# wq2012/SpectralCluster

Hardware: AMD Instinct MI355X
Metric: predict() calls/sec, n=8192 d=256 ICASSP2018 (GraphCut, eigengap k in [2,20], cosine k-means) (higher is better)
Workload: dtype f64; 1 GPU; icassp2018_graphcut_n8192_d256_k8_max20; n_samples=8192, n_features=256, parallelism=replicas x1, collectives=none

## Files before the change

spectralcluster_amd/csrc/eig.hip:

```cpp
#include <algorithm>
#include <cstring>
#include <mutex>

#include "sc_internal.h"

namespace sc {

typedef double v4f64 __attribute__((ext_vector_type(4)));
constexpr int B = kEigBlock;
constexpr int RB = 256 / B;
static_assert(B == 8 || B == 16, "block width must divide the 16-wide MFMA tile");

__device__ __forceinline__ uint64_t splitmix64(uint64_t x) {
  x += 0x9E3779B97F4A7C15ull;
  x = (x ^ (x >> 30)) * 0xBF58476D1CE4E5B9ull;
  x = (x ^ (x >> 27)) * 0x94D049BB133111EBull;
  return x ^ (x >> 31);
}
__device__ __forceinline__ double hash_uniform(uint64_t seed, uint64_t idx) {
  const uint64_t h = splitmix64(seed ^ splitmix64(idx));
  return (double)(h >> 11) * (2.0 / 9007199254740992.0) - 1.0;
}

__global__ void k_random_block(double* W, int n, uint64_t seed) {
  const int e = blockIdx.x * blockDim.x + threadIdx.x;
  if (e < n * B) W[e] = hash_uniform(seed, (uint64_t)e);
}

__global__ void k_refill_deficient(double* W, int n, const int* flags,
                                   uint64_t seed) {
  const int e = blockIdx.x * blockDim.x + threadIdx.x;
  if (e >= n * B) return;
  if ((flags[0] >> (e & (B - 1))) & 1) W[e] = hash_uniform(seed, (uint64_t)e);
}

constexpr int kMvWaves = 8;
__device__ __forceinline__ void block_matvec_body(
    const double* __restrict__ S, int ld, int n, const double* __restrict__ cvec,
    const double* __restrict__ pvec, const double* __restrict__ V, int ldv,
    const double* __restrict__ Vs, double* __restrict__ W) {
  __shared__ double red[kMvWaves][64][4];
  const int lane = threadIdx.x & 63;
  const int wave = threadIdx.x >> 6;
  const int li = lane & 15, lg = lane >> 4;
  const int r0 = blockIdx.x * 16;
  int ri = r0 + li;
  ri = ri < n ? ri : n - 1;
  const double* srow = S + (size_t)ri * ld + 2 * lg;
  v4f64 acc0 = {0.0, 0.0, 0.0, 0.0}, acc1 = {0.0, 0.0, 0.0, 0.0};
  const int nchunks = (n + 31) / 32;
  double2 cur[4], nxt[4];
  auto load = [&](double2* dst, int ch) {
    const int kb = ch * 32 + 2 * lg;
#pragma unroll
    for (int q = 0; q < 4; ++q) {
      if (kb + 8 * q + 1 < ld)
        dst[q] = *reinterpret_cast<const double2*>(srow + ch * 32 + 8 * q);
      else
        dst[q] = make_double2(0.0, 0.0);
    }
  };
  int ch = wave;
  if (ch < nchunks) load(cur, ch);
  for (; ch < nchunks; ch += kMvWaves) {
    if (ch + kMvWaves < nchunks) load(nxt, ch + kMvWaves);
    const int kb = ch * 32 + 2 * lg;
    double b[8];
#pragma unroll
    for (int t = 0; t < 8; ++t) {
      const int k = kb + 8 * (t >> 1) + (t & 1);
      b[t] = (k < n && li < B) ? Vs[(size_t)k * B + li] : 0.0;
    }
#pragma unroll
    for (int q = 0; q < 4; ++q) {
      const double a0 = (kb + 8 * q < n) ? cur[q].x : 0.0;
      const double a1 = (kb + 8 * q + 1 < n) ? cur[q].y : 0.0;
      acc0 = __builtin_amdgcn_mfma_f64_16x16x4f64(a0, b[2 * q], acc0, 0, 0, 0);
      acc1 = __builtin_amdgcn_mfma_f64_16x16x4f64(a1, b[2 * q + 1], acc1, 0, 0, 0);
    }
#pragma unroll
    for (int q = 0; q < 4; ++q) cur[q] = nxt[q];
  }
#pragma unroll
  for (int r = 0; r < 4; ++r) red[wave][lane][r] = acc0[r] + acc1[r];
  __syncthreads();
  if (wave == 0) {
#pragma unroll
    for (int r = 0; r < 4; ++r) {
      double sum = 0.0;
#pragma unroll
      for (int w = 0; w < kMvWaves; ++w) sum += red[w][lane][r];
      const int row = r0 + lg + 4 * r;
      if (row < n && li < B)
        W[(size_t)row * B + li] =
            __builtin_fma(cvec ? cvec[row] : 1.0, sum,
                          pvec ? pvec[row] * V[(size_t)row * ldv + li] : 0.0);
    }
  }
}
__global__ __launch_bounds__(64 * kMvWaves) void k_block_matvec(
    const double* __restrict__ S, int ld, int n, const double* __restrict__ cvec,
    const double* __restrict__ pvec, const double* __restrict__ V, int ldv,
    const double* __restrict__ Vs, double* __restrict__ W) {
  block_matvec_body(S, ld, n, cvec, pvec, V, ldv, Vs, W);
}
__global__ __launch_bounds__(64 * kMvWaves) void k_block_matvec_g(const GroupOf<MatvecItem> g) {
  const MatvecItem& a = g.s[blockIdx.y];
  if ((int)blockIdx.x * 16 >= a.n) return;
  block_matvec_body(a.S, a.ld, a.n, a.cvec, a.pvec, a.V, a.ldv, a.Vs, a.W);
}

constexpr int kSymTile = 128;
constexpr int kSymPitch = 34;
__device__ __forceinline__ int sym_item_id(int I, int J, int nt) {
  return I * nt - I * (I - 1) / 2 + (J - I);
}
__device__ __forceinline__ void block_matvec_sym_body(
    const double* __restrict__ S, int ld, int n, const double* __restrict__ Vs,
    double* __restrict__ pdirect, double* __restrict__ pmirror, int nt) {
  __shared__ __attribute__((aligned(16))) double smem[4 * 32 * kSymPitch];
  int I = 0, rem = blockIdx.x, rowlen = nt;
  while (rem >= rowlen) {
    rem -= rowlen;
    --rowlen;
    ++I;
  }
  const int J = I + rem;
  const bool diag = I == J;
  const int lane = threadIdx.x & 63, wave = threadIdx.x >> 6;
  const int li = lane & 15, lg = lane >> 4;
  const int r0 = I * kSymTile + 32 * wave;
  const int c0 = J * kSymTile;
  double* patch = smem + wave * (32 * kSymPitch);
  double bm[8];
#pragma unroll
  for (int t = 0; t < 8; ++t) {
    const int row = r0 + 4 * t + lg;
    bm[t] = (row < n && li < B) ? Vs[(size_t)row * B + li] : 0.0;
  }
  v4f64 accd[2] = {{0.0, 0.0, 0.0, 0.0}, {0.0, 0.0, 0.0, 0.0}};
  v4f64 accm[4][2];
#pragma unroll
  for (int cs = 0; cs < 4; ++cs)
#pragma unroll
    for (int ct = 0; ct < 2; ++ct) accm[cs][ct] = (v4f64){0.0, 0.0, 0.0, 0.0};
  double2 a[1][2][4];
  auto load = [&](int buf, int cs) {
#pragma unroll
    for (int rt = 0; rt < 2; ++rt) {
      int row = r0 + 16 * rt + li;
      row = row < n ? row : n - 1;
      const double* src = S + (size_t)row * ld + c0 + 32 * cs + 2 * lg;
#pragma unroll
      for (int q = 0; q < 4; ++q) {
        if (c0 + 32 * cs + 8 * q + 2 * lg + 1 < ld)
          a[buf][rt][q] = *reinterpret_cast<const double2*>(src + 8 * q);
        else
          a[buf][rt][q] = make_double2(0.0, 0.0);
      }
    }
  };
#pragma unroll
  for (int cs = 0; cs < 4; ++cs) {
    constexpr int cur = 0;
    load(cur, cs);
    const int kb = c0 + 32 * cs + 2 * lg;
#pragma unroll
    for (int rt = 0; rt < 2; ++rt) {
      const bool rok = r0 + 16 * rt + li < n;
#pragma unroll
      for (int q = 0; q < 4; ++q) {
        if (!rok || kb + 8 * q >= n) a[cur][rt][q].x = 0.0;
        if (!rok || kb + 8 * q + 1 >= n) a[cur][rt][q].y = 0.0;
      }
    }
    double b[8];
#pragma unroll
    for (int t = 0; t < 8; ++t) {
      const int k = kb + 8 * (t >> 1) + (t & 1);
      b[t] = (k < n && li < B) ? Vs[(size_t)k * B + li] : 0.0;
    }
#pragma unroll
    for (int rt = 0; rt < 2; ++rt)
#pragma unroll
      for (int q = 0; q < 4; ++q) {
        accd[rt] = __builtin_amdgcn_mfma_f64_16x16x4f64(a[cur][rt][q].x, b[2 * q], accd[rt], 0, 0, 0);
        accd[rt] = __builtin_amdgcn_mfma_f64_16x16x4f64(a[cur][rt][q].y, b[2 * q + 1], accd[rt], 0, 0, 0);
      }
    if (!diag) {
#pragma unroll
      for (int rt = 0; rt < 2; ++rt)
#pragma unroll
        for (int q = 0; q < 4; ++q)
          *reinterpret_cast<double2*>(patch + (16 * rt + li) * kSymPitch + 8 * q + 2 * lg) =
              a[cur][rt][q];
      __builtin_amdgcn_fence(__ATOMIC_RELEASE, "wavefront");
      __builtin_amdgcn_wave_barrier();
#pragma unroll
      for (int ct = 0; ct < 2; ++ct)
#pragma unroll
        for (int t = 0; t < 8; ++t) {
          const double at = patch[(4 * t + lg) * kSymPitch + 16 * ct + li];
          accm[cs][ct] = __builtin_amdgcn_mfma_f64_16x16x4f64(at, bm[t], accm[cs][ct], 0, 0, 0);
        }
      __builtin_amdgcn_fence(__ATOMIC_ACQUIRE, "wavefront");
      __builtin_amdgcn_wave_barrier();
    }
  }
  const size_t item = blockIdx.x;
  if (li < B) {
#pragma unroll
    for (int rt = 0; rt < 2; ++rt)
#pragma unroll
      for (int r = 0; r < 4; ++r)
        pdirect[(item * kSymTile + 32 * wave + 16 * rt + lg + 4 * r) * B + li] = accd[rt][r];
  }
  if (diag) return;
  __syncthreads();
  double* red = smem;
  if (li < B) {
#pragma unroll
    for (int cs = 0; cs < 4; ++cs)
#pragma unroll
      for (int ct = 0; ct < 2; ++ct)
#pragma unroll
        for (int r = 0; r < 4; ++r)
          red[(wave * kSymTile + 32 * cs + 16 * ct + lg + 4 * r) * B + li] = accm[cs][ct][r];
  }
  __syncthreads();
  for (int e = threadIdx.x; e < kSymTile * B; e += 256)
    pmirror[item * (kSymTile * B) + e] =
        ((red[e] + red[kSymTile * B + e]) + red[2 * kSymTile * B + e]) + red[3 * kSymTile * B + e];
}
__global__ __launch_bounds__(256) void k_block_matvec_sym(
    const double* __restrict__ S, int ld, int n, const double* __restrict__ Vs,
    double* __restrict__ pdirect, double* __restrict__ pmirror, int nt) {
  block_matvec_sym_body(S, ld, n, Vs, pdirect, pmirror, nt);
}
__global__ __launch_bounds__(256) void k_block_matvec_sym_g(const GroupOf<MatvecItem> g) {
  const MatvecItem& a = g.s[blockIdx.y];
  const int nt = (a.n + kSymTile - 1) / kSymTile;
  if ((int)blockIdx.x >= nt * (nt + 1) / 2) return;
  block_matvec_sym_body(a.S, a.ld, a.n, a.Vs, a.slabs, a.slabs + (size_t)(nt * (nt + 1) / 2) * kSymTile * B, nt);
}

__device__ __forceinline__ void matvec_sym_reduce_body(
    const double* __restrict__ pdirect, const double* __restrict__ pmirror, int nt, int n,
    const double* __restrict__ cvec, const double* __restrict__ pvec,
    const double* __restrict__ V, int ldv, double* __restrict__ W) {
  const int R = blockIdx.x / 4;
  const int e = (blockIdx.x & 3) * 256 + threadIdx.x;
  const int rl = e / B, v = e % B;
  const int row = R * kSymTile + rl;
  double acc = 0.0;
  const int total = nt;
  for (int s0 = 0; s0 < total; s0 += 8) {
    double x[8];
#pragma unroll
    for (int u = 0; u < 8; ++u) {
      const int sidx = s0 + u;
      x[u] = 0.0;
      if (sidx < nt - R) {
        x[u] = pdirect[(size_t)sym_item_id(R, R + sidx, nt) * (kSymTile * B) + e];
      } else if (sidx < total) {
        x[u] = pmirror[(size_t)sym_item_id(sidx - (nt - R), R, nt) * (kSymTile * B) + e];
      }
    }
#pragma unroll
    for (int u = 0; u < 8; ++u) acc += x[u];
  }
  if (row < n) W[(size_t)row * B + v] =
      __builtin_fma(cvec ? cvec[row] : 1.0, acc, pvec ? pvec[row] * V[(size_t)row * ldv + v] : 0.0);
}
__global__ __launch_bounds__(256) void k_matvec_sym_reduce(
    const double* __restrict__ pdirect, const double* __restrict__ pmirror, int nt, int n,
    const double* __restrict__ cvec, const double* __restrict__ pvec,
    const double* __restrict__ V, int ldv, double* __restrict__ W) {
  matvec_sym_reduce_body(pdirect, pmirror, nt, n, cvec, pvec, V, ldv, W);
}
__global__ __launch_bounds__(256) void k_matvec_sym_reduce_g(const GroupOf<MatvecItem> g) {
  const MatvecItem& a = g.s[blockIdx.y];
  const int nt = (a.n + kSymTile - 1) / kSymTile;
  if ((int)blockIdx.x >= nt * 4) return;
  matvec_sym_reduce_body(a.slabs, a.slabs + (size_t)(nt * (nt + 1) / 2) * kSymTile * B, nt, a.n,
                         a.cvec, a.pvec, a.V, a.ldv, a.W);
}

constexpr int kProjGroups = 256 / B;
constexpr int kProjAcc = (kLdq + kProjGroups - 1) / kProjGroups;
__global__ __launch_bounds__(256) void k_proj_partial(
    const double* __restrict__ Q, int ldq, int m, const double* __restrict__ W,
    int n, double* __restrict__ partial) {
  __shared__ double Ql[8][kLdq];
  __shared__ double Wl[8][B];
  const int tid = threadIdx.x;
  const int jj = tid % B, ig = tid / B;
  const int rows_per = (n + gridDim.x - 1) / gridDim.x;
  const int rbeg = blockIdx.x * rows_per;
  const int rend = min(n, rbeg + rows_per);
  double acc[kProjAcc];
#pragma unroll
  for (int q = 0; q < kProjAcc; ++q) acc[q] = 0.0;
  for (int r = rbeg; r < rend; r += 8) {
    __syncthreads();
    for (int e = tid; e < 8 * m; e += 256) {
      const int rr = e / m, i = e - rr * m;
      Ql[rr][i] = (r + rr < rend) ? Q[(size_t)(r + rr) * ldq + i] : 0.0;
    }
    if (tid < 8 * B) {
      const int rr = tid / B;
      Wl[rr][jj] = (r + rr < rend) ? W[(size_t)(r + rr) * B + jj] : 0.0;
    }
    __syncthreads();
#pragma unroll
    for (int rr = 0; rr < 8; ++rr) {
      const double w = Wl[rr][jj];
#pragma unroll
      for (int q = 0; q < kProjAcc; ++q)
        if (ig + kProjGroups * q < m)
          acc[q] = __builtin_fma(Ql[rr][ig + kProjGroups * q], w, acc[q]);
    }
  }
  double* out = partial + (size_t)blockIdx.x * (kLdq * B);
#pragma unroll
  for (int q = 0; q < kProjAcc; ++q)
    if (ig + kProjGroups * q < m) out[(ig + kProjGroups * q) * B + jj] = acc[q];
}

__global__ __launch_bounds__(256) void k_reduce_H(
    const double* __restrict__ partial, int nparts, int m, double* __restrict__ Hbuf,
    double* __restrict__ T, int ldt, int col0, int accumulate,
    double* __restrict__ hsq) {
  __shared__ double sq[32];
  const int tid = threadIdx.x;
  const int sub = tid & 7;
  const int e = blockIdx.x * 32 + (tid >> 3);
  double h = 0.0;
  if (e < m * B)
    for (int g = sub; g < nparts; g += 8) h += partial[(size_t)g * (kLdq * B) + e];
  h += __shfl_xor(h, 1);
  h += __shfl_xor(h, 2);
  h += __shfl_xor(h, 4);
  if (sub == 0) {
    if (e < m * B) {
      Hbuf[e] = h;
      if (T != nullptr) {
        const int i = e / B, j = col0 + (e % B);
        if (i <= j) {
          const double v = accumulate ? T[(size_t)i * ldt + j] + h : h;
          T[(size_t)i * ldt + j] = v;
          T[(size_t)j * ldt + i] = v;
        }
      }
    } else {
      h = 0.0;
    }
    sq[tid >> 3] = h * h;
  }
  __syncthreads();
  if (tid < B) {
    double s = 0.0;
    for (int q = tid; q < 32; q += B) s += sq[q];
    atomicAdd(&hsq[tid], s);
  }
}

__global__ __launch_bounds__(256) void k_update_block(
    const double* __restrict__ Q, int ldq, int m, const double* __restrict__ Hbuf,
    double* __restrict__ W, int n) {
  __shared__ double Hl[kLdq * B];
  __shared__ double Ql[RB][kLdq + 1];
  const int tid = threadIdx.x;
  const int jj = tid % B, rr = tid / B;
  const int r0 = blockIdx.x * RB;
  for (int e = tid; e < m * B; e += 256) Hl[e] = Hbuf[e];
  for (int e = tid; e < RB * m; e += 256) {
    const int a = e / m, i = e - a * m;
    Ql[a][i] = (r0 + a < n) ? Q[(size_t)(r0 + a) * ldq + i] : 0.0;
  }
  __syncthreads();
  const int r = r0 + rr;
  if (r < n) {
    double acc = W[(size_t)r * B + jj];
    for (int i = 0; i < m; ++i) acc = __builtin_fma(-Ql[rr][i], Hl[i * B + jj], acc);
    W[(size_t)r * B + jj] = acc;
  }
}

__device__ __forceinline__ void chol8_wave(const double* G, double* __restrict__ Rinv,
                                           const double* __restrict__ hsq,
                                           int* __restrict__ flags,
                                           int* __restrict__ defect_flag, int flag_mode,
                                           int* __restrict__ sticky_flag = nullptr,
                                           int sticky_m = 0, bool sticky_on_defect = true);

__global__ __launch_bounds__(256) void k_reduce_chol(
    const double* __restrict__ partial, int nparts, double* __restrict__ Rinv,
    double* __restrict__ Gsave, const double* __restrict__ hsq,
    int* __restrict__ flags, int* __restrict__ defect_flag, int flag_mode) {
  static_assert(B == 8, "the factorisation below maps the 8 x 8 matrix onto one wavefront");
  __shared__ double G[B * B];
  const int tid = threadIdx.x;
  {
    constexpr int kLanes = 256 / (B * B);
    const int e = tid / kLanes, sub = tid % kLanes;
    double g = 0.0;
    for (int q = sub; q < nparts; q += kLanes) g += partial[(size_t)q * (kLdq * B) + e];
#pragma unroll
    for (int o = 1; o < kLanes; o <<= 1) g += __shfl_xor(g, o);
    if (sub == 0) {
      G[e] = g;
      if (Gsave) Gsave[e] = g;
    }
  }
  __syncthreads();
  if (tid >= 64) return;
  chol8_wave(G, Rinv, hsq, flags, defect_flag, flag_mode);
}

__device__ __forceinline__ void chol8_wave(const double* G, double* __restrict__ Rinv,
                                           const double* __restrict__ hsq,
                                           int* __restrict__ flags,
                                           int* __restrict__ defect_flag, int flag_mode,
                                           int* __restrict__ sticky_flag, int sticky_m,
                                           bool sticky_on_defect) {
  const int tid = threadIdx.x;
  const int i = tid >> 3, j = tid & 7;
  double g = G[tid];
  const double gii = __shfl(g, i * 9), gjj = __shfl(g, j * 9);
  double defect = 0.0;
  if (flag_mode == 2 && gii != 0.0 && gjj != 0.0) defect = fabs(g - (i == j ? 1.0 : 0.0));
#pragma unroll
  for (int o = 1; o < 64; o <<= 1) defect = fmax(defect, __shfl_xor(defect, o));
  double r = 0.0;
  int mask = 0;
  double pmax = 0.0, pmin = __builtin_huge_val();
#pragma unroll
  for (int k = 0; k < B; ++k) {
    const double d = __shfl(g, k * 9);
    const double total = __shfl(gii, k * 8) + (hsq ? hsq[k] : 0.0);
    const bool drop = !(d > 1e-22 * total) || !(d > 0.0);
    const double rk = drop ? 0.0 : sqrt(d);
    if (drop) {
      mask |= 1 << k;
    } else {
      pmax = fmax(pmax, rk);
      pmin = fmin(pmin, rk);
    }
    double row = 0.0;
    if (i == k && !drop) row = j == k ? rk : (j > k ? g / rk : 0.0);
    if (i == k) r = row;
    const double rki = __shfl(row, k * 8 + i), rkj = __shfl(row, k * 8 + j);
    if (i > k && j > k) g -= rki * rkj;
  }
  const double rii = __shfl(r, i * 9), rjj = __shfl(r, j * 9);
  double ri = 0.0;
#pragma unroll
  for (int srow = B - 1; srow >= 0; --srow) {
    double v = 0.0;
#pragma unroll
    for (int k = srow + 1; k < B; ++k) {
      const double rsk = __shfl(r, srow * 8 + k), rkj = __shfl(ri, k * 8 + j);
      if (k <= j) v -= rsk * rkj;
    }
    if (i == srow && j >= i && rii != 0.0 && rjj != 0.0)
      ri = i == j ? 1.0 / rii : v / rii;
  }
  Rinv[tid] = ri;
  if (tid == 0 && flags != nullptr) {
    flags[0] = mask;
    if (defect_flag != nullptr) *defect_flag = (defect > 0.1 || pmax > 1e3 * pmin) ? 1 : 0;
    if (sticky_flag != nullptr && (mask != 0 || (sticky_on_defect && defect > 0.1))) {
      if (*sticky_flag == 0) {
        sticky_flag[1] = sticky_m;
        sticky_flag[2] = flag_mode * 1000 + mask;
      }
      *sticky_flag = 1;
    }
  }
}

__global__ __launch_bounds__(256) void k_apply_rinv(
    double* __restrict__ W, int n, const double* __restrict__ Rinv,
    double* __restrict__ Qdst, int ldq, int col0, const double* __restrict__ cvec,
    double* __restrict__ Vs) {
  __shared__ double Rl[B * B];
  const int tid = threadIdx.x;
  if (tid < B * B) Rl[tid] = Rinv[tid];
  __syncthreads();
  const int jj = tid % B;
  const int r = blockIdx.x * RB + tid / B;
  const double w = r < n ? W[(size_t)r * B + jj] : 0.0;
  double v = 0.0;
#pragma unroll
  for (int k = 0; k < B; ++k) {
    const double wk = __shfl(w, k, B);
    v = __builtin_fma(wk, Rl[k * B + jj], v);
  }
  if (r < n) {
    W[(size_t)r * B + jj] = v;
    if (Qdst) Qdst[(size_t)r * ldq + col0 + jj] = v;
    if (Vs) Vs[(size_t)r * B + jj] = cvec[r] * v;
  }
}

constexpr int kLzThreads = 512;
constexpr int kLzPartStride = (kLdq + B) * B;
struct LzStep {
  double* W;
  int n;
  const double* Q;
  int ldq, m;
  int pre;
  const double* pre_partial;
  int pre_nparts;
  double* T;
  int ldt, col0;
  double* Gsave;
  double* hsq;
  int* flags;
  int arm_defect;
  double* Tzero;
  double* Qdst;
  int store_col;
  const double* vs_scale;
  double* Vs;
  int init_random;
  uint64_t seed;
  int want_proj, want_gram;
  double* partial;
};

__device__ __forceinline__ double lz_ordered_sum(const double* src, int nparts) {
  double acc = 0.0;
  for (int p0 = 0; p0 < nparts; p0 += 16) {
    double v[16];
#pragma unroll
    for (int u = 0; u < 16; ++u)
      v[u] = (p0 + u < nparts) ? src[(size_t)(p0 + u) * kLzPartStride] : 0.0;
#pragma unroll
    for (int u = 0; u < 16; ++u) acc += v[u];
  }
// ... 845 lines not shown
```

Measured before the change: 390.4 calls/s.

## Stream symmetric block-matvec tiles through an LDS ring via direct global-to-LDS loads

```diff
diff --git a/spectralcluster_amd/csrc/eig.hip b/spectralcluster_amd/csrc/eig.hip
--- a/spectralcluster_amd/csrc/eig.hip
+++ b/spectralcluster_amd/csrc/eig.hip
@@ -1,6 +1,7 @@
 #include <algorithm>
 #include <cstring>
 #include <mutex>
+#include <type_traits>
 
 #include "sc_internal.h"
 
@@ -111,14 +112,121 @@
 }
 
 constexpr int kSymTile = 128;
-constexpr int kSymPitch = 34;
+constexpr int kSymStageCols = 16;
+constexpr int kSymStageRows = 16;
+constexpr int kSymDepth = 3;
+constexpr int kSymColParts = 32 / kSymStageCols;
+constexpr int kSymRowParts = 32 / kSymStageRows;
+constexpr int kSymStages = 4 * kSymColParts * kSymRowParts;
+constexpr int kSymCpr = kSymStageCols / 2;
+constexpr int kSymStageDoubles = kSymStageRows * kSymStageCols;
+constexpr int kSymGlds = kSymStageDoubles * 8 / 1024;
+constexpr int kSymRing = 4 * kSymDepth * kSymStageDoubles;
+constexpr int kSymRed = 4 * kSymTile * B;
+constexpr int kSymLds = kSymRing + kSymTile * B > kSymRed ? kSymRing + kSymTile * B : kSymRed;
+static_assert(B == 8, "the Vs tile is staged as 128 rows of 64 bytes");
+static_assert(kSymStageRows == 16 || kSymStageRows == 32, "a stage holds whole direct tiles");
+static_assert(kSymGlds >= 1 && kSymGlds * 128 == kSymStageDoubles, "whole DMA instructions");
+static_assert(kSymDepth >= 2 && kSymDepth <= kSymStages, "ring depth");
+static_assert(kSymGlds * (kSymDepth - 1) <= 4, "sym_wait_vmcnt knows the counts 0, 2 and 4");
+static_assert(kSymLds * sizeof(double) <= 65536, "static LDS");
+constexpr __host__ __device__ int sym_key(int row) {
+  return (row >> 1) & 7;
+}
+constexpr __host__ __device__ int sym_slot(int row, int chunk) {
+  return row * kSymCpr + (chunk ^ sym_key(row));
+}
+constexpr __host__ __device__ int sym_slot_row(int slot) { return slot / kSymCpr; }
+constexpr __host__ __device__ int sym_slot_chunk(int slot) {
+  return (slot % kSymCpr) ^ sym_key(slot / kSymCpr);
+}
+constexpr __host__ __device__ int sym_direct_off(int row, int col) {
+  return 2 * sym_slot(row, col >> 1);
+}
+constexpr __host__ __device__ int sym_mirror_off(int row, int col) {
+  return 2 * sym_slot(row, col >> 1) + (col & 1);
+}
+constexpr __host__ __device__ int sym_mirror_lane_base(int i, int g, int t_and_3) {
+  return 2 * (g * kSymCpr + (((i >> 1) ^ (g >> 1)) ^ (2 * t_and_3))) + (i & 1);
+}
+constexpr __host__ __device__ int sym_mirror_step(int t) { return 2 * (4 * t) * kSymCpr; }
+constexpr bool sym_mirror_split_agrees() {
+  for (int t = 0; t < kSymStageRows / 4; ++t)
+    for (int g = 0; g < 4; ++g)
+      for (int i = 0; i < 16; ++i)
+        if (sym_mirror_lane_base(i, g, t & 3) + sym_mirror_step(t) != sym_mirror_off(4 * t + g, i))
+          return false;
+  return true;
+}
+constexpr bool sym_maps_agree() {
+  for (int slot = 0; slot < kSymStageRows * kSymCpr; ++slot) {
+    const int row = sym_slot_row(slot), chunk = sym_slot_chunk(slot);
+    if (row < 0 || row >= kSymStageRows || chunk < 0 || chunk >= kSymCpr) return false;
+    if (sym_slot(row, chunk) != slot) return false;
+    if (sym_direct_off(row, 2 * chunk) != 2 * slot) return false;
+    if (sym_mirror_off(row, 2 * chunk) != 2 * slot) return false;
+    if (sym_mirror_off(row, 2 * chunk + 1) != 2 * slot + 1) return false;
+  }
+  for (int row = 0; row < kSymStageRows; ++row)
+    for (int chunk = 0; chunk < kSymCpr; ++chunk) {
+      const int slot = sym_slot(row, chunk);
+      if (slot < 0 || slot >= kSymStageRows * kSymCpr) return false;
+      if (sym_slot_row(slot) != row || sym_slot_chunk(slot) != chunk) return false;
+    }
+  return true;
+}
+constexpr bool sym_direct_conflict_free() {
+  for (int rt = 0; rt < kSymStageRows / 16; ++rt)
+    for (int chunk = 0; chunk < kSymCpr; ++chunk) {
+      unsigned seen = 0;
+      for (int li = 0; li < 16; ++li) seen |= 1u << (sym_slot(16 * rt + li, chunk) & 15);
+      if (seen != 0xFFFFu) return false;
+    }
+  return true;
+}
+constexpr bool sym_mirror_conflict_free() {
+  for (int t = 0; t < kSymStageRows / 4; ++t)
+    for (int ct = 0; ct < kSymStageCols / 16; ++ct)
+      for (int half = 0; half < 2; ++half) {
+        unsigned seen = 0;
+        for (int g = 2 * half; g < 2 * half + 2; ++g)
+          for (int i = 0; i < 16; ++i) seen |= 1u << (sym_mirror_off(4 * t + g, 16 * ct + i) & 31);
+        if (seen != 0xFFFFFFFFu) return false;
+      }
+  return true;
+}
+static_assert(sym_maps_agree(), "both read maps return the element the DMA put there");
+static_assert(sym_mirror_split_agrees(), "lane base + step is the mirror read map");
+static_assert(sym_direct_conflict_free(), "direct ds_read_b128: 16 lanes, 16 bank groups");
+static_assert(sym_mirror_conflict_free(), "mirror ds_read_b64: 32 lanes, 32 bank pairs");
+
+constexpr __host__ __device__ int sym_stage_strip(int st) {
+  return st / (kSymColParts * kSymRowParts);
+}
+constexpr __host__ __device__ int sym_stage_col0(int st) {
+  return 32 * sym_stage_strip(st) + kSymStageCols * ((st / kSymRowParts) % kSymColParts);
+}
+constexpr __host__ __device__ int sym_stage_row0(int st) {
+  return kSymStageRows * (st % kSymRowParts);
+}
 __device__ __forceinline__ int sym_item_id(int I, int J, int nt) {
   return I * nt - I * (I - 1) / 2 + (J - I);
+}
+__device__ __forceinline__ void sym_glds16(const double* g, double* l) {
+  __builtin_amdgcn_global_load_lds((const __attribute__((address_space(1))) void*)(g),
+                                   (__attribute__((address_space(3))) void*)(l), 16, 0, 0);
+}
+__device__ __forceinline__ void sym_wait_vmcnt(int count) {
+  switch (count) {
+    case 2: asm volatile("s_waitcnt vmcnt(2)" ::: "memory"); break;
+    case 4: asm volatile("s_waitcnt vmcnt(4)" ::: "memory"); break;
+    default: asm volatile("s_waitcnt vmcnt(0)" ::: "memory"); break;
+  }
 }
 __device__ __forceinline__ void block_matvec_sym_body(
     const double* __restrict__ S, int ld, int n, const double* __restrict__ Vs,
     double* __restrict__ pdirect, double* __restrict__ pmirror, int nt) {
-  __shared__ __attribute__((aligned(16))) double smem[4 * 32 * kSymPitch];
+  __shared__ __attribute__((aligned(16))) double smem[kSymLds];
   int I = 0, rem = blockIdx.x, rowlen = nt;
   while (rem >= rowlen) {
     rem -= rowlen;
@@ -127,86 +235,106 @@
   }
   const int J = I + rem;
   const bool diag = I == J;
-  const int lane = threadIdx.x & 63, wave = threadIdx.x >> 6;
+  const int lane = threadIdx.x & 63;
+  const int wave = __builtin_amdgcn_readfirstlane(threadIdx.x >> 6);
   const int li = lane & 15, lg = lane >> 4;
   const int r0 = I * kSymTile + 32 * wave;
   const int c0 = J * kSymTile;
-  double* patch = smem + wave * (32 * kSymPitch);
+  double* ring = smem + wave * (kSymDepth * kSymStageDoubles);
+  double* vsj = smem + kSymRing;
+#pragma unroll
+  for (int u = 0; u < 2; ++u) {
+    const int ch = 64 * (2 * wave + u) + lane;
+    int row = c0 + (ch >> 2);
+    row = row < n ? row : n - 1;
+    sym_glds16(Vs + (size_t)row * B + 2 * (ch & 3), vsj + 128 * (2 * wave + u));
+  }
+  auto issue = [&](int stage, bool clamp) {
+    double* dst = ring + (stage % kSymDepth) * kSymStageDoubles;
+#pragma unroll
+    for (int j = 0; j < kSymGlds; ++j) {
+      const int slot = 64 * j + lane;
+      int row = r0 + sym_stage_row0(stage) + sym_slot_row(slot);
+      int col = c0 + sym_stage_col0(stage) + 2 * sym_slot_chunk(slot);
+      if (clamp) {
+        row = row < n ? row : n - 1;
+        col = col < ld - 2 ? col : ld - 2;
+      }
+      sym_glds16(S + (size_t)row * ld + col, dst + 128 * j);
+    }
+  };
+#pragma unroll
+  for (int st = 0; st < kSymDepth; ++st) issue(st, true);
   double bm[8];
 #pragma unroll
   for (int t = 0; t < 8; ++t) {
     const int row = r0 + 4 * t + lg;
-    bm[t] = (row < n && li < B) ? Vs[(size_t)row * B + li] : 0.0;
-  }
+    const double x = Vs[(size_t)(row < n ? row : n - 1) * B + (li & (B - 1))];
+    bm[t] = (row < n && li < B) ? x : 0.0;
+  }
+  sym_wait_vmcnt(0);
+  __syncthreads();
   v4f64 accd[2] = {{0.0, 0.0, 0.0, 0.0}, {0.0, 0.0, 0.0, 0.0}};
   v4f64 accm[4][2];
 #pragma unroll
   for (int cs = 0; cs < 4; ++cs)
 #pragma unroll
     for (int ct = 0; ct < 2; ++ct) accm[cs][ct] = (v4f64){0.0, 0.0, 0.0, 0.0};
-  double2 a[1][2][4];
-  auto load = [&](int buf, int cs) {
-#pragma unroll
-    for (int rt = 0; rt < 2; ++rt) {
-      int row = r0 + 16 * rt + li;
-      row = row < n ? row : n - 1;
-      const double* src = S + (size_t)row * ld + c0 + 32 * cs + 2 * lg;
-#pragma unroll
-      for (int q = 0; q < 4; ++q) {
-        if (c0 + 32 * cs + 8 * q + 2 * lg + 1 < ld)
-          a[buf][rt][q] = *reinterpret_cast<const double2*>(src + 8 * q);
-        else
-          a[buf][rt][q] = make_double2(0.0, 0.0);
+  int mbase[4];
+#pragma unroll
+  for (int c = 0; c < 4; ++c) mbase[c] = sym_mirror_lane_base(li, lg, c);
+  auto stream = [&](auto edge_tag) {
+    constexpr bool kEdge = decltype(edge_tag)::value;
+#pragma unroll
+    for (int st = 0; st < kSymStages; ++st) {
+      const int ahead = kSymStages - 1 - st < kSymDepth - 1 ? kSymStages - 1 - st : kSymDepth - 1;
+      sym_wait_vmcnt(kSymGlds * ahead);
+      const double* buf = ring + (st % kSymDepth) * kSymStageDoubles;
+      const int cs = sym_stage_strip(st);
+      const int cb = sym_stage_col0(st);
+      const int rb = sym_stage_row0(st);
+#pragma unroll
+      for (int qq = 0; qq < kSymStageCols / 8; ++qq) {
+        const int kl = cb + 8 * qq + 2 * lg;
+        const int k = c0 + kl;
+        double b0 = vsj[kl * B + (li & (B - 1))];
+        double b1 = vsj[(kl + 1) * B + (li & (B - 1))];
+        b0 = (!kEdge || k < n) ? b0 : 0.0;
+        b1 = (!kEdge || k + 1 < n) ? b1 : 0.0;
+#pragma unroll
+        for (int rl = 0; rl < kSymStageRows / 16; ++rl) {
+          const int rt = rb / 16 + rl;
+          const bool rok = !kEdge || r0 + 16 * rt + li < n;
+          const double2 a = *reinterpret_cast<const double2*>(
+              buf + sym_direct_off(16 * rl + li, 8 * qq + 2 * lg));
+          const double ax = (!rok || (kEdge && k >= n)) ? 0.0 : a.x;
+          const double ay = (!rok || (kEdge && k + 1 >= n)) ? 0.0 : a.y;
+          accd[rt] = __builtin_amdgcn_mfma_f64_16x16x4f64(ax, b0, accd[rt], 0, 0, 0);
+          accd[rt] = __builtin_amdgcn_mfma_f64_16x16x4f64(ay, b1, accd[rt], 0, 0, 0);
+        }
       }
-    }
-  };
-#pragma unroll
-  for (int cs = 0; cs < 4; ++cs) {
-    constexpr int cur = 0;
-    load(cur, cs);
-    const int kb = c0 + 32 * cs + 2 * lg;
-#pragma unroll
-    for (int rt = 0; rt < 2; ++rt) {
-      const bool rok = r0 + 16 * rt + li < n;
-#pragma unroll
-      for (int q = 0; q < 4; ++q) {
-        if (!rok || kb + 8 * q >= n) a[cur][rt][q].x = 0.0;
-        if (!rok || kb + 8 * q + 1 >= n) a[cur][rt][q].y = 0.0;
-      }
-    }
-    double b[8];
-#pragma unroll
-    for (int t = 0; t < 8; ++t) {
-      const int k = kb + 8 * (t >> 1) + (t & 1);
-      b[t] = (k < n && li < B) ? Vs[(size_t)k * B + li] : 0.0;
-    }
-#pragma unroll
-    for (int rt = 0; rt < 2; ++rt)
-#pragma unroll
-      for (int q = 0; q < 4; ++q) {
-        accd[rt] = __builtin_amdgcn_mfma_f64_16x16x4f64(a[cur][rt][q].x, b[2 * q], accd[rt], 0, 0, 0);
-        accd[rt] = __builtin_amdgcn_mfma_f64_16x16x4f64(a[cur][rt][q].y, b[2 * q + 1], accd[rt], 0, 0, 0);
-      }
-    if (!diag) {
-#pragma unroll
-      for (int rt = 0; rt < 2; ++rt)
-#pragma unroll
-        for (int q = 0; q < 4; ++q)
-          *reinterpret_cast<double2*>(patch + (16 * rt + li) * kSymPitch + 8 * q + 2 * lg) =
-              a[cur][rt][q];
-      __builtin_amdgcn_fence(__ATOMIC_RELEASE, "wavefront");
-      __builtin_amdgcn_wave_barrier();
-#pragma unroll
-      for (int ct = 0; ct < 2; ++ct)
-#pragma unroll
-        for (int t = 0; t < 8; ++t) {
-          const double at = patch[(4 * t + lg) * kSymPitch + 16 * ct + li];
+      if (!diag) {
+        const int ct = (cb % 32) / 16;
+        const bool cok = !kEdge || c0 + cb + li < n;
+#pragma unroll
+        for (int tl = 0; tl < kSymStageRows / 4; ++tl) {
+          const int t = rb / 4 + tl;
+          const bool ok = cok && (!kEdge || r0 + 4 * t + lg < n);
+          const double x = buf[mbase[tl & 3] + sym_mirror_step(tl)];
+          const double at = ok ? x : 0.0;
           accm[cs][ct] = __builtin_amdgcn_mfma_f64_16x16x4f64(at, bm[t], accm[cs][ct], 0, 0, 0);
         }
-      __builtin_amdgcn_fence(__ATOMIC_ACQUIRE, "wavefront");
-      __builtin_amdgcn_wave_barrier();
-    }
-  }
+      }
+      if (st + kSymDepth < kSymStages) {
+        asm volatile("s_waitcnt lgkmcnt(0)" ::: "memory");
+        issue(st + kSymDepth, kEdge);
+      }
+    }
+  };
+  if (c0 + kSymTile > n)
+    stream(std::true_type{});
+  else
+    stream(std::false_type{});
   const size_t item = blockIdx.x;
   if (li < B) {
 #pragma unroll
@@ -232,12 +360,13 @@
     pmirror[item * (kSymTile * B) + e] =
         ((red[e] + red[kSymTile * B + e]) + red[2 * kSymTile * B + e]) + red[3 * kSymTile * B + e];
 }
-__global__ __launch_bounds__(256) void k_block_matvec_sym(
+#define SC_SYM_OCC __attribute__((amdgpu_waves_per_eu(4, 4)))
+__global__ __launch_bounds__(256) SC_SYM_OCC void k_block_matvec_sym(
     const double* __restrict__ S, int ld, int n, const double* __restrict__ Vs,
     double* __restrict__ pdirect, double* __restrict__ pmirror, int nt) {
   block_matvec_sym_body(S, ld, n, Vs, pdirect, pmirror, nt);
 }
-__global__ __launch_bounds__(256) void k_block_matvec_sym_g(const GroupOf<MatvecItem> g) {
+__global__ __launch_bounds__(256) SC_SYM_OCC void k_block_matvec_sym_g(const GroupOf<MatvecItem> g) {
   const MatvecItem& a = g.s[blockIdx.y];
   const int nt = (a.n + kSymTile - 1) / kSymTile;
   if ((int)blockIdx.x >= nt * (nt + 1) / 2) return;
```

Measured after the change: 402.0 calls/s (median of 6 runs). +3.0%, better.
